# micropilot/myosuite-mjx

Hardware: AMD Instinct MI355X
Metric: env-steps/s (whole node) myoHandPoseRandom-v0 batch 4096 (higher is better)
Workload: dtype f32

## Files before the change

myosuite_mjx_amd/csrc/myo_common.h:

```cpp
#ifndef MYO_COMMON_H
#define MYO_COMMON_H

#include <hip/hip_runtime.h>

#include <algorithm>
#include <utility>
#include <cmath>
#include <cstdint>
#include <cstdio>
#include <cstdlib>
#include <cstring>
#include <mutex>
#include <string>
#include <vector>

#include "../../include/myo_hip.h"

#define MINVALF 1e-15f
#define MAXVALF 1e10f
#define MINIMPF 0.0001f
#define MAXIMPF 0.9999f
#define NCON 32
#define NCAND 128
#ifndef LS_FLOOR
// ... 116 lines not shown

struct TaskDev {
  int task, frame_skip, reset_random, target_generate, ntarget, ntip, obs_dim, nq;
  int tip_site[8];
  float pose_thd, far_th, near_th, w_pose, w_bonus, w_act_reg, w_penalty, w_reach;
  const float *target_lo, *target_hi, *init_qpos, *jnt_lo, *jnt_hi;
  const float* init_qvel;
  const float* rnd;
  float tip_lpos[3];
  int gsize_type;
  float gsize_lo[3], gsize_hi[3];
  const float *init_qpos_alt, *init_qvel_alt;
  float reset_noise_std;
  int fatigue_mode;
  const float* fatigue_vec;
  int terrain, hf_n;
  float terrain_lo, terrain_hi;
  float bd_frame[12];
};

struct DevWalk {
  int obs_dim, hip_period;
  float dt, min_height, max_rot, target_x_vel, target_y_vel;
  float target_rot[4];
  int link_tl, link_tr, link_pel, link_tor;
  float lpos_tl[3], lpos_tr[3], lpos_pel[3], lquat_tor[4];
  int qadr_hfl, qadr_hfr, qadr_ja[4];
  float w_vel, w_done, w_cyc, w_rot, w_ja;
  float mass_total, static_mcom[3];
  float knee_height;
};
enum { KF_AUX = 1, KF_OBS_ONLY = 2, KF_RESET_ONLY = 4 };

__device__ __forceinline__ float dot3(const float* a, const float* b) { return a[0] * b[0] + a[1] * b[1] + a[2] * b[2]; }
__device__ __forceinline__ void cross3(float* r, const float* a, const float* b) {
  float x = a[1] * b[2] - a[2] * b[1], y = a[2] * b[0] - a[0] * b[2], z = a[0] * b[1] - a[1] * b[0];
  r[0] = x; r[1] = y; r[2] = z;
}
__device__ __forceinline__ float norm3(const float* a) { return sqrtf(dot3(a, a)); }
__device__ __forceinline__ float normalize3(float* a) {
  float n = norm3(a);
  if (n < MINVALF) { a[0] = 1; a[1] = 0; a[2] = 0; } else { float i = 1.0f / n; a[0] *= i; a[1] *= i; a[2] *= i; }
  return n;
}
__device__ __forceinline__ float clipf(float x, float lo, float hi) { return fminf(fmaxf(x, lo), hi); }
__device__ __forceinline__ void quat2mat(float* R, const float* q) {
  float w = q[0], x = q[1], y = q[2], z = q[3];
  R[0] = w * w + x * x - y * y - z * z; R[1] = 2 * (x * y - w * z); R[2] = 2 * (x * z + w * y);
  R[3] = 2 * (x * y + w * z); R[4] = w * w - x * x + y * y - z * z; R[5] = 2 * (y * z - w * x);
  R[6] = 2 * (x * z - w * y); R[7] = 2 * (y * z + w * x); R[8] = w * w - x * x - y * y + z * z;
}
__device__ __forceinline__ void euler2quat(float* q, const float* e) {
  float si, ci, sj, cj, sk, ck;
  sincosf(0.5f * e[2], &si, &ci);
  sincosf(-0.5f * e[1], &sj, &cj);
  sincosf(0.5f * e[0], &sk, &ck);
  const float cc = ci * ck, cs = ci * sk, sc = si * ck, ss = si * sk;
  q[0] = cj * cc + sj * ss;
  q[1] = cj * cs - sj * sc;
  q[2] = -(cj * ss + sj * cc);
  q[3] = cj * sc - sj * cs;
}
__device__ __forceinline__ void mulquat(float* r, const float* a, const float* b) {
  float t0 = a[0] * b[0] - a[1] * b[1] - a[2] * b[2] - a[3] * b[3];
  float t1 = a[0] * b[1] + a[1] * b[0] + a[2] * b[3] - a[3] * b[2];
  float t2 = a[0] * b[2] - a[1] * b[3] + a[2] * b[0] + a[3] * b[1];
// ... 83 lines not shown
```

myosuite_mjx_amd/csrc/myo_hip.hip:

```cpp
#include "myo_common.h"
#include "myo_physics.h"
#include "myo_task_track.h"
#include "myo_kernel_lanes.h"
#include "myo_kernel_wave.h"
#include "myo_kernels_aux.h"
#include "myo_host.h"
#include "myo_task_keyturn.h"
#include "myo_task_pen.h"
#include "myo_task_baoding.h"
#include "myo_task_die.h"
#include "myo_task_myodm.h"
#include "myo_host_model.h"

extern "C" {

const char* myo_last_error(void) { return g_err.c_str(); }
int myo_version(void) { return 1; }

int myo_model_load(const void* blobv, size_t nbytes, int device, myo_model** out) {
  if (!blobv || !out || nbytes < 16) return fail(MYO_E_ARG, "myo_model_load: bad arguments");
  const Blob B{(const uint8_t*)blobv};
  uint32_t ver;
  memcpy(&ver, B.p + 4, 4);
  if (memcmp(B.p, "MYOB", 4) || ver != 3) return fail(MYO_E_BLOB, "myo_model_load: not a MYOB v3 blob");
// ... 552 lines not shown
  if (!b) return fail(MYO_E_ARG, "null batch");
  b->env_offset = env_offset;
  b->db.env_offset = env_offset;
  return MYO_OK;
}

int myo_set_state(myo_batch* b, const float* qpos, const float* qvel, const float* act, const float* time, void* stream) {
  if (!b) return fail(MYO_E_ARG, "myo_set_state: null");
  const DevModel& dm = b->model->dm;
  size_t B = b->db.B;
  hipStream_t s = (hipStream_t)stream;
  if (qpos) HIPCHK(hipMemcpyAsync(b->db.qpos, qpos, B * b->model->nq * 4, hipMemcpyDeviceToDevice, s));
  if (qvel) HIPCHK(hipMemcpyAsync(b->db.qvel, qvel, B * dm.nv * 4, hipMemcpyDeviceToDevice, s));
  if (act) HIPCHK(hipMemcpyAsync(b->db.act, act, B * dm.nu * 4, hipMemcpyDeviceToDevice, s));
  if (time) HIPCHK(hipMemcpyAsync(b->db.time, time, B * 4, hipMemcpyDeviceToDevice, s));
  return MYO_OK;
}

#define MYO_WAVE_KERNELS(X)                                                                                             \
  X(WK_HAND, "step_kernel_w<24,8,32,1,3,false,0,false>", 24, 8, 32, 1, 3, false, 0)                                      \
  X(WK_HAND_SPEC, "step_kernel_w<24,8,32,1,4,false,1,false>", 24, 8, 32, 1, 4, false, 1)                                 \
  X(WK_LEG, "step_kernel_w<36,20,32,2,2,false,0,false>", 36, 20, 32, 2, 2, false, 0)                                     \
  X(WK_LEG_SCHED, "step_kernel_w<36,20,32,2,2,true,0,false>", 36, 20, 32, 2, 2, true, 0)                                 \
  X(WK_LEG_SPEC_SCHED, "step_kernel_w<36,20,32,2,2,true,2,false>", 36, 20, 32, 2, 2, true, 2)                            \
  X(WK_LEG_SPEC, "step_kernel_w<36,20,32,2,2,false,2,false>", 36, 20, 32, 2, 2, false, 2)                                \
  X(WK_TERRAIN, "step_kernel_w<36,20,32,2,2,false,0,true>", 36, 20, 32, 2, 2, false, 0, true)                            \
  X(WK_TERRAIN_SPEC_SCHED, "step_kernel_w<36,20,32,2,2,true,3,true>", 36, 20, 32, 2, 2, true, 3, true)                   \
  X(WK_TERRAIN_SPEC, "step_kernel_w<36,20,32,2,2,false,3,true>", 36, 20, 32, 2, 2, false, 3, true)                       \
  X(WK_TRK, "step_kernel_w<36,20,32,2,2,false,0,false,true>", 36, 20, 32, 2, 2, false, 0, false, true)                   \
  X(WK_HAND_RK4, "step_kernel_w<24,8,32,1,3,false,0,false,false,true>", 24, 8, 32, 1, 3, false, 0, false, false, true)   \
  X(WK_LEG_RK4, "step_kernel_w<36,20,32,2,2,false,0,false,false,true>", 36, 20, 32, 2, 2, false, 0, false, false, true)
struct WaveKernel {
  const char* name;
  void (*fn)(const DevModel*, const DevModelW*, DevBatch, const float*, int, int, long long*, const int*, const DevWalk*, int, SchedDev);
};
enum WaveKernelId {
#define X(id, name, ...) id,
  MYO_WAVE_KERNELS(X)
#undef X
};
static const WaveKernel wave_kernels[] = {
#define X(id, name, ...) {name, step_kernel_w<__VA_ARGS__>},
  MYO_WAVE_KERNELS(X)
#undef X
};

static WaveKernelId select_wave_kernel(const myo_model* m, bool bm, bool sched) {
  const bool hand_sizes = m->hand_sizes && !bm, leg_sizes = m->leg_sizes && !bm;
  if (sched) return m->dw.hf.on ? WK_TERRAIN_SPEC_SCHED : (leg_sizes ? WK_LEG_SPEC_SCHED : WK_LEG_SCHED);
  if (m->rk4) return m->wave_cfg == 0 ? WK_HAND_RK4 : WK_LEG_RK4;
  if (m->wave_cfg == 2) return WK_TRK;
  if (m->wave_cfg == 0) return hand_sizes ? WK_HAND_SPEC : WK_HAND;
  if (m->dw.hf.on) return m->terrain_sizes ? WK_TERRAIN_SPEC : WK_TERRAIN;
  return leg_sizes ? WK_LEG_SPEC : WK_LEG;
}

static int launch_step(myo_batch* b, const float* action, int actmap, int nsub, hipStream_t s, int kflags = 0) {
  const myo_model* m = b->model;
  const DevWalk* wk = b->task.task == MYO_TASK_WALK ? b->d_walk : nullptr;
  if (kflags && !(wk && g_lanes == 64)) return fail(MYO_E_ARG, "observation pass: walk task on the wave kernel only");
  const int G = (g_lanes == 64 && !m->wave_ok) ? 16 : ((g_lanes != 64 && !m->generic_ok) ? 64 : g_lanes), EPW = 64 / G;
  int grid = (b->db.B + EPW - 1) / EPW;
  size_t lds = (size_t)EPW * m->env_lds_bytes;
  {
    static std::mutex attr_g_mu;
    static bool attr_g_dev[64] = {};
    std::lock_guard<std::mutex> attr_g_lock(attr_g_mu);
    bool& attr_set = attr_g_dev[m->device & 63];
    if (!attr_set) {
      for (const void* k : {(const void*)step_kernel<16>, (const void*)step_kernel<32>, (const void*)step_kernel<64>, (const void*)reach_obs_kernel<16>})
        HIPCHK(hipFuncSetAttribute(k, hipFuncAttributeMaxDynamicSharedMemorySize, 160 * 1024));
      attr_set = true;
    }
  }
  long long* st = b->d_stamps;
#if MYO_POISON
  {
    static const int pmode = [] { const char* e = getenv("MYO_POISON_MODE"); return e ? atoi(e) : 7; }();
    if (pmode & 1) hipLaunchKernelGGL(scratch_poison_kernel, dim3(16384), dim3(64), 0, s, (float*)b->d_stamps, 0);
    if (pmode & 2) hipLaunchKernelGGL(vgpr_poison_kernel, dim3(8192), dim3(64), 0, s, 0x7fc0dead);
    if (pmode & 4) hipLaunchKernelGGL(sgpr_poison_kernel, dim3(32768), dim3(64), 0, s);
  }
#endif
  if (!(G == 64 && m->wave_ok) && !m->generic_ok)
    return fail(MYO_E_UNSUPPORTED, "this model (tendon limits / free joint / equalities / plane contacts) needs the wave-per-env kernel (lanes = 64)");
  const bool bm = b->bm_on;
  if (bm) {
    int rc = bm_check(b);
    if (rc) return rc;
    const int n = b->db.B * m->dm.nl;
    hipLaunchKernelGGL(link_compose_kernel, dim3((n + 255) / 256), dim3(256), 0, s, b->db, m->dm.nl, m->d_lm_adr, m->d_lm_body, m->d_lm_tab);
// ... 1 lines not shown
  if (G == 64 && m->wave_ok) {
    static std::mutex attr_mu;
    static bool attr_w_dev[64] = {};
    std::lock_guard<std::mutex> attr_lock(attr_mu);
    bool& attr_w = attr_w_dev[m->device & 63];
    if (!attr_w) {
      for (const WaveKernel& k : wave_kernels) HIPCHK(hipFuncSetAttribute((const void*)k.fn, hipFuncAttributeMaxDynamicSharedMemorySize, 64 * 1024));
      attr_w = true;
    }
    const int* order = nullptr;
    int Bn = b->db.B;
    static const int sched_mode = [] { const char* e = getenv("MYO_SCHED"); return e ? atoi(e) : -1; }();
    const int n_cu = m->n_cu > 0 ? m->n_cu : 256;
    const int resident = n_cu * (m->wave_cfg == 0 ? 16 : (m->wave_cfg == 1 ? 8 : std::max(1, (160 * 1024) / std::max(1, m->env_lds_bytes_w))));
    const bool sched_ok = !kflags && Bn >= 64 && Bn <= SCHED_ENV_MASK && nsub + (wk ? 1 : 0) <= 15 && nsub > 0;
    const bool sched = sched_ok && !bm && m->wave_cfg == 1 && !m->rk4 && !(m->dw.hf.on && !m->terrain_sizes) && (sched_mode == 1 || (sched_mode == -1 && m->wave_cfg == 1 && Bn >= 2 * resident));
    if (b->balance && Bn >= 1024 && Bn % 4 == 0 && !kflags && !sched) {
      static const int prio_mode = [] { const char* e = getenv("MYO_PRIO"); return e ? atoi(e) : 2; }();
      hipLaunchKernelGGL(balance_kernel, dim3(1), dim3(1024), 0, s, (const int*)b->db.diag, Bn, b->d_order, Bn / 4, prio_mode);
      order = b->d_order;
    }
    const int nqueue = std::max(1, std::min(8, n_cu / 32));
    SchedDev S{b->d_sched, b->d_sched + 32, nqueue == 8 ? b->sched_stride : (Bn + nqueue - 1) / nqueue + 1, nsub + (wk ? 1 : 0), nqueue};
    const WaveKernel& k = wave_kernels[select_wave_kernel(m, bm, sched)];
    if (!kflags) b->last_kernel = k.name;
    int wgrid = Bn;
    if (sched) {
      hipLaunchKernelGGL(sched_init_kernel, dim3(1), dim3(1024), 0, s, (const int*)b->db.diag, Bn, S);
      wgrid = Bn < resident ? Bn : resident;
      static const int grid_override = [] { const char* e = getenv("MYO_SCHED_GRID"); return e ? atoi(e) : 0; }();
      if (grid_override > 0 && grid_override < wgrid) wgrid = grid_override;
    }
    hipLaunchKernelGGL(k.fn, dim3(wgrid), dim3(64), (size_t)m->env_lds_bytes_w, s, (const DevModel*)m->d_dm, (const DevModelW*)m->d_dw, b->db, action, actmap,
                       nsub, st, order, wk, kflags, S);
    HIPCHK(hipGetLastError());
    return MYO_OK;
  }
  if (G == 16) hipLaunchKernelGGL(step_kernel<16>, dim3(grid), dim3(64), lds, s, m->dm, b->db, action, actmap, nsub, st);
  else if (G == 32) hipLaunchKernelGGL(step_kernel<32>, dim3(grid), dim3(64), lds, s, m->dm, b->db, action, actmap, nsub, st);
  else hipLaunchKernelGGL(step_kernel<64>, dim3(grid), dim3(64), lds, s, m->dm, b->db, action, actmap, nsub, st);
  HIPCHK(hipGetLastError());
  return MYO_OK;
}

int myo_step(myo_batch* b, const float* action_dev, int actmap, int nsubsteps, void* stream) {
  if (!b || nsubsteps < 0) return fail(MYO_E_ARG, "myo_step: bad arguments");
  if (b->task.task == MYO_TASK_TRACK && b->track_flavour == 1 && actmap == MYO_ACTMAP_CTRLRANGE)
    return fail(MYO_E_ARG, "myo_step: MYO_ACTMAP_CTRLRANGE is the MJX TrackEnv's action map; a batch of the classic flavour steps with MYO_ACTMAP_MUSCLE_SIGMOID");
  HIPCHK(hipSetDevice(b->model->device));
  return launch_step(b, action_dev, actmap, nsubsteps, (hipStream_t)stream);
}

static int state_configure(myo_batch* b, const myo_task_config* c) {
  const myo_model* m = b->model;
  const int nv = m->dm.nv, nq = m->nq, na = m->dm.na_obs;
  if (c->task == MYO_TASK_POSE) {
    if (c->ntarget != nv) return fail(MYO_E_ARG, "pose task: ntarget must equal nq");
    b->task.obs_dim = 3 * nv + na;
  } else if (c->task == MYO_TASK_STAND) {
    if (c->ntarget != 3) return fail(MYO_E_ARG, "stand task: ntarget must be 3 (target position)");
    if (!(m->wave_ok && m->dw.has_free && nq == nv + 1)) return fail(MYO_E_UNSUPPORTED, "stand task needs a model with a free root joint");
    b->task.obs_dim = nq + nv + 6 + na;
  } else {
    if (c->ntarget != 3) return fail(MYO_E_ARG, "hold task: ntarget must be 3 (goal position)");
    if (!(m->wave_ok && m->dw.has_free && nq == nv + 1 && nv > 6)) return fail(MYO_E_UNSUPPORTED, "hold task needs a model whose last joint is one free object");
    b->task.obs_dim = (nq - 7) + (nv - 6) + 6 + na;
  }
// ... 94 lines not shown
  HIPCHK(hipGetLastError());
  return MYO_OK;
}

int myo_set_balance(myo_batch* b, int on) {
  if (!b) return fail(MYO_E_ARG, "null batch");
  b->balance = on;
  return MYO_OK;
}

int myo_set_lanes(int lanes) {
  if (lanes != 16 && lanes != 32 && lanes != 64) return fail(MYO_E_ARG, "lanes per env must be 16, 32 or 64");
  g_lanes = lanes;
  return MYO_OK;
}

int myo_read_stamps(myo_batch* b, long long* host, int nwg) {
  if (!b || !host) return fail(MYO_E_ARG, "myo_read_stamps: null");
  HIPCHK(hipDeviceSynchronize());
  HIPCHK(hipMemcpy(host, b->d_stamps, (size_t)nwg * 12 * sizeof(long long), hipMemcpyDeviceToHost));
  return MYO_STAMPS ? MYO_OK : 1;
}

int myo_sync(void* stream) {
  HIPCHK(hipStreamSynchronize((hipStream_t)stream));
  return MYO_OK;
}

int myo_bench_rollout(myo_batch* b, int steps, int nsubsteps, uint64_t seed, int mode, int max_episode_steps, void* stream, float* ms_out) {
  if (!b || steps <= 0) return fail(MYO_E_ARG, "myo_bench_rollout: bad arguments");
  HIPCHK(hipSetDevice(b->model->device));
  hipStream_t s = (hipStream_t)stream;
  int rc;
  if (!(mode & MYO_BENCH_FRESH_ACTIONS)) { rc = myo_random_action(b, b->d_action, seed, b->bench_step, b->env_offset, stream); if (rc) return rc; }
  const int base = ms_out ? 0 : b->kev_pending;
  while ((int)b->kev.size() < 2 * (base + steps)) { hipEvent_t e; HIPCHK(hipEventCreate(&e)); b->kev.push_back(e); }
  if (ms_out) { b->kev_pending = 0; HIPCHK(hipEventRecord(b->ev0, s)); }
  for (int i = 0; i < steps; i++) {
    if (mode & MYO_BENCH_FRESH_ACTIONS) { rc = myo_random_action(b, b->d_action, seed, b->bench_step++, b->env_offset, stream); if (rc) return rc; }
    HIPCHK(hipEventRecord(b->kev[2 * (base + i)], s));
    const bool mjx_track = b->task.task == MYO_TASK_TRACK && b->track_flavour == 0;
    rc = launch_step(b, b->d_action, mjx_track ? MYO_ACTMAP_CTRLRANGE : MYO_ACTMAP_MUSCLE_SIGMOID, nsubsteps, s);
    if (rc) return rc;
    HIPCHK(hipEventRecord(b->kev[2 * (base + i) + 1], s));
    const TaskHooks* hooks = task_hooks(b->task.task);
    if (mjx_track) continue;
    if ((mode & MYO_BENCH_OBS) && (mode & MYO_BENCH_AUTORESET) && max_episode_steps > 0 && hooks && hooks->post) {
      if ((rc = hooks->post(b, s, seed, max_episode_steps))) return rc;
      HIPCHK(hipGetLastError());
      continue;
    }
    if ((mode & MYO_BENCH_OBS) && b->task.task != MYO_TASK_NONE && b->task.task != MYO_TASK_WALK) { rc = launch_obs(b, s); if (rc) return rc; }
    if ((mode & MYO_BENCH_AUTORESET) && max_episode_steps > 0) {
      rc = myo_autoreset(b, max_episode_steps, seed, stream); if (rc) return rc;
      if ((mode & MYO_BENCH_OBS) && b->task.task != MYO_TASK_NONE) { rc = launch_obs(b, s, 1, 1); if (rc) return rc; }
    }
  }
  if (!ms_out) { b->kev_pending = base + steps; return MYO_OK; }
  HIPCHK(hipEventRecord(b->ev1, s));
  HIPCHK(hipEventSynchronize(b->ev1));
  HIPCHK(hipEventElapsedTime(ms_out, b->ev0, b->ev1));
  float tot = 0.f;
  for (int i = 0; i < steps; i++) { float t; HIPCHK(hipEventElapsedTime(&t, b->kev[2 * i], b->kev[2 * i + 1])); tot += t; }
  b->last_kernel_ms = tot;
  return MYO_OK;
}

const char* myo_bench_last_kernel_name(const myo_batch* b) { return b ? b->last_kernel : ""; }

int myo_probe_valu(int device, int waves_per_simd, int iters, double* wave_insts_per_s, int* n_cu_out) {
  if (!wave_insts_per_s || !(waves_per_simd >= 1 && waves_per_simd <= 4 || waves_per_simd == 8) || iters < 1) return fail(MYO_E_ARG, "myo_probe_valu: waves_per_simd must be 1..4 or 8");
  HIPCHK(hipSetDevice(device));
  hipDeviceProp_t prop;
  HIPCHK(hipGetDeviceProperties(&prop, device));
  const int ncu = prop.multiProcessorCount;
  const size_t lds = 60 * 1024;
  HIPCHK(hipFuncSetAttribute((const void*)valu_probe_kernel, hipFuncAttributeMaxDynamicSharedMemorySize, 64 * 1024));
  float* out = nullptr;
  const int wg_per_cu = waves_per_simd == 8 ? 2 : 1;
// ... 92 lines not shown
```

myosuite_mjx_amd/csrc/myo_kernel_wave.h:

```cpp
#ifndef MYO_KERNEL_WAVE_H
#define MYO_KERNEL_WAVE_H

#define NCONW 32
#define MPRW 14
static_assert(4 * MPRW <= 63, "the scheduler carries the table in a 64-word row (word 63 = entry count)");
struct LayW {
  int qpos, qvel, act, ctrl, lpos, lmat, axis, anchor, xv, qfc, sq, mprw, X;
  int tJ, tlen, tforce;
  int cdof, cinert, crb, cvel, cacc, cfrc;
  int gpos, gax, cand, cdist, cpos, cnrm, cpair, cJ, cdofs;
  int Mp;
  int tJp;
  int total;
};
__host__ __device__ constexpr LayW layout_w(int nq, int nv, int nu, int nl, int ngt, int maxnnz, int ncg, bool has_tl, int nvt, int kc, int nc, int nj) {
  LayW Y{};
  int o = 0;
  Y.qpos = o; o += nq; Y.qvel = o; o += nv; Y.act = o; o += nu; Y.ctrl = o; o += nu;
  Y.lpos = o; o += 3 * nl; Y.lmat = o; o += 9 * nl; Y.axis = o; o += 3 * nv; Y.anchor = o; o += 3 * nv;
  Y.xv = o; o += nvt; Y.qfc = o; o += nvt; Y.sq = o; o += nvt * (nvt + 1); Y.mprw = o; o += 4 * MPRW;
  Y.tJp = 0;
  if (has_tl) { Y.tJp = o; o += ngt * maxnnz + 2 * ngt; }
  Y.X = o;
  Y.tJ = o; o += ngt * maxnnz; Y.tlen = o; o += ngt; Y.tforce = o; o += nu;
// ... 313 lines not shown
  __syncthreads();
  if (t == 0) { int acc = 0; for (int k = 0; k < 256; k++) { start[k] = acc; acc += hist[k]; } }
  __syncthreads();
  for (int e = t; e < B; e += 1024) {
    int b = 255 - min(255, (int)(255LL * diag[(size_t)e * 8 + 3] / cmax));
    int r = atomicAdd(&start[b], 1);
    S.ring[(r % nqu) * S.stride + r / nqu] = e;
  }
}

template <int SPEC> struct Sizes { static constexpr int nq = 0, nv = 0, nu = 0, nl = 0, nlevel = 0, maxnnz = 0, nseg = 0, ncg = 0, npair = 0; };
template <> struct Sizes<1> { static constexpr int nq = 23, nv = 23, nu = 39, nl = 17, nlevel = 5, maxnnz = 7, nseg = 116, ncg = 27, npair = 289; };
template <> struct Sizes<2> { static constexpr int nq = 35, nv = 34, nu = 80, nl = 13, nlevel = 6, maxnnz = 11, nseg = 100, ncg = 32, npair = 45; };
template <> struct Sizes<3> { static constexpr int nq = 35, nv = 34, nu = 80, nl = 13, nlevel = 6, maxnnz = 11, nseg = 100, ncg = 33, npair = 76; };
template <int SPEC> static bool sizes_match(int nq, int nv, int nu, int nl, int nlevel, int maxnnz, int ngt, int nseg, int ncg, int npair) {
  typedef Sizes<SPEC> Z;
  return nq == Z::nq && nv == Z::nv && nu == Z::nu && nl == Z::nl && nlevel == Z::nlevel && maxnnz == Z::maxnnz && ngt == Z::nu && nseg == Z::nseg &&
         ncg == Z::ncg && npair == Z::npair;
}

template <int SPEC, int NVT, int KC, int NC, int NJ> struct LayC {
  typedef Sizes<SPEC> Z;
  static constexpr LayW L = layout_w(Z::nq, Z::nv, Z::nu, Z::nl, Z::nu, Z::maxnnz, Z::ncg, false, NVT, KC, NC, NJ);
  static constexpr int qpos = L.qpos, qvel = L.qvel, act = L.act, ctrl = L.ctrl, lpos = L.lpos, lmat = L.lmat, axis = L.axis, anchor = L.anchor, xv = L.xv,
                       qfc = L.qfc, sq = L.sq, mprw = L.mprw, X = L.X, tJ = L.tJ, tlen = L.tlen, tforce = L.tforce, cdof = L.cdof, cinert = L.cinert, crb = L.crb,
                       cvel = L.cvel, cacc = L.cacc, cfrc = L.cfrc, gpos = L.gpos, gax = L.gax, cand = L.cand, cdist = L.cdist, cpos = L.cpos, cnrm = L.cnrm,
                       cpair = L.cpair, cJ = L.cJ, cdofs = L.cdofs, Mp = L.Mp, tJp = L.tJp, total = L.total;
};
template <int SPEC, int NVT, int KC, int NC, int NJ> static bool layout_match(const LayW& a) {
  const LayW b = layout_w(Sizes<SPEC>::nq, Sizes<SPEC>::nv, Sizes<SPEC>::nu, Sizes<SPEC>::nl, Sizes<SPEC>::nu, Sizes<SPEC>::maxnnz, Sizes<SPEC>::ncg, false, NVT, KC, NC, NJ);
  return memcmp(&a, &b, sizeof(LayW)) == 0;
}

template <int NVT, int KC, int NC, int NTR, int WPE, bool SCHED, int SPEC, bool HF = false, bool TRK = false, bool RK4 = false>
__global__ void __launch_bounds__(64, WPE) step_kernel_w(const DevModel* __restrict__ Mp, const DevModelW* __restrict__ Wp, DevBatch Bt,
                                                        const float* __restrict__ action, int actmap, int nsub, long long* stamps,
                                                        const int* __restrict__ order, const DevWalk* __restrict__ wk, int kflags, SchedDev S) {
  extern __shared__ __align__(16) float E[];
  const DevModel& M = *Mp;
  const DevModelW& W = *Wp;
  const LayC<SPEC, NVT, KC, NC, (TRK ? 4 : 3)> Yc{};
  const auto& Y = [&]() -> const auto& { if constexpr (SPEC != 0) return Yc; else return W.lay; }();
#define lane_id wave_lane()
  const int oe = (!SCHED && order) ? order[blockIdx.x] : blockIdx.x;
  int env = oe & 0x0FFFFFFF;
  if (!SCHED) {
    switch (oe >> 28) {
      case 3: __builtin_amdgcn_s_setprio(3); break;
      case 2: __builtin_amdgcn_s_setprio(2); break;
      case 1: __builtin_amdgcn_s_setprio(1); break;
      default: break;
    }
  }
  typedef Sizes<SPEC> Z;
  const int nv = SPEC ? Z::nv : M.nv, nu = SPEC ? Z::nu : M.nu, nq = SPEC ? Z::nq : W.nq;
  const int nl_ = SPEC ? Z::nl : M.nl, nlevel_ = SPEC ? Z::nlevel : M.nlevel, maxnnz_ = SPEC ? Z::maxnnz : M.maxnnz, ngt_ = SPEC ? Z::nu : M.ngt,
            nseg_ = SPEC ? Z::nseg : M.nseg, ncg_ = SPEC ? Z::ncg : M.ncg, npair_ = SPEC ? Z::npair : M.npair;
  constexpr int CDW = (KC + 3) / 4;
  constexpr int NJ = TRK ? 4 : 3;
  constexpr int NR = TRK ? 6 : 4;
  constexpr bool FULL = NVT > 24;
  const bool has_free = FULL && W.has_free;
  const int neq = FULL ? W.neq : 0;
  const bool has_tl = (SPEC != 0 || TRK) ? false : (W.has_tl != 0);
  const bool walk = FULL && wk != nullptr;
  if (!SCHED && FULL && (kflags & KF_RESET_ONLY) && Bt.elapsed[env] != 0) return;
#if MYO_STAMPS
  long long st_acc[12] = {0, 0, 0, 0, 0, 0, 0, 0, 0, 0, 0, 0};
  long long st_t0 = clock64();
  long long st_sub[12] = {0, 0, 0, 0, 0, 0, 0, 0, 0, 0, 0, 0}, st_s0 = 0;
  long long st_x[12] = {0, 0, 0, 0, 0, 0, 0, 0, 0, 0, 0, 0};
#define SUB0() do { st_s0 = clock64(); } while (0)
#define SUB(k) do { long long t1_ = clock64(); st_sub[k] += t1_ - st_s0; st_s0 = t1_; } while (0)
#define SUBX(k) do { long long t1_ = clock64(); st_x[k] += t1_ - st_s0; st_s0 = t1_; } while (0)
#define CNTX(k) do { st_x[k]++; } while (0)
#else
#define SUB0() do { } while (0)
#define SUB(k) do { } while (0)
#define SUBX(k) do { } while (0)
#define CNTX(k) do { } while (0)
#endif
  const int nsubtot = nsub + (walk ? 1 : 0);
  const float h = M.timestep;
  const int sq_q = SCHED ? (int)(__builtin_amdgcn_s_getreg((31 << 11) | 20) & 7) % S.nqueue : 0;
  int* const sq_ctl = SCHED ? S.ctl + 4 * sq_q : nullptr;
  int* const sq_ring = SCHED ? S.ring + (size_t)sq_q * S.stride : nullptr;
  const int sq_n = SCHED ? sq_ctl[2] : 0;
  int last_cost = 0;
  for (;;) {
  int s0 = 0, s1 = nsubtot;
  if (SCHED) {
    int t = 0;
    if (lane_id == 0) t = atomicAdd(&sq_ctl[0], 1);
    t = __builtin_amdgcn_readfirstlane(t);
    if (t >= sq_n * nsubtot) break;
    const int gen = t / sq_n, slot = t - gen * sq_n;
    int v = 0, spins = 0;
    for (;;) {
      v = __hip_atomic_load(&sq_ring[slot], __ATOMIC_RELAXED, __HIP_MEMORY_SCOPE_AGENT);
      if ((v >> 24) == gen || ++spins > (1 << 21)) break;
      __builtin_amdgcn_s_sleep(8);
    }
    v = __builtin_amdgcn_readfirstlane(v);
    if ((v >> 24) != gen) { if (lane_id == 0) { atomicOr(&Bt.flags[0], MYO_FLAG_SCHED_TIMEOUT); sq_ctl[3] = 1; } break; }
    env = v & SCHED_ENV_MASK;
    s0 = (v >> 20) & 15; s1 = s0 + 1;
  }
  float actdot[NTR];
  float* const warm_row = Bt.warm + (size_t)env * nv;
#pragma unroll
  for (int r = 0; r < NTR; r++) actdot[r] = 0.f;
#ifndef MYO_POISON_BITS
#define MYO_POISON_BITS 0x7fc00000
#endif
#if MYO_POISON
  { const int lo_ = MYO_POISON == 1 ? 0 : MYO_POISON == 2 ? 0 : MYO_POISON == 3 ? Y.xv : MYO_POISON == 4 ? Y.sq : MYO_POISON == 5 ? Y.mprw : Y.X;
    const int hi_ = MYO_POISON == 1 ? Y.total : MYO_POISON == 2 ? Y.xv : MYO_POISON == 3 ? Y.sq : MYO_POISON == 4 ? Y.mprw : MYO_POISON == 5 ? Y.X : Y.total;
    for (int i = lo_ + lane_id; i < hi_; i += 64) E[i] = __int_as_float(MYO_POISON_BITS); }
  SYNC();
#endif
  if (lane_id < nq) E[Y.qpos + lane_id] = ldstate<SCHED>(Bt.qpos + (size_t)env * nq + lane_id);
  if (lane_id < nv) {
    E[Y.qvel + lane_id] = ldstate<SCHED>(Bt.qvel + (size_t)env * nv + lane_id);
  }
  for (int i = lane_id; i < nu; i += 64) {
    E[Y.act + i] = ldstate<SCHED>(Bt.act + (size_t)env * nu + i);
    float c;
    if (action && s0 == 0) c = action_map(Bt, M.act, action, env, i, nu, actmap);
    else c = ldstate<SCHED>(Bt.ctrl + (size_t)env * nu + i);
    E[Y.ctrl + i] = c;
  }
  float time = uniformf(ldstate<SCHED>(Bt.time + env));
  const bool track_on = TRK && Bt.track != nullptr && action != nullptr && actmap == MYO_ACTMAP_CTRLRANGE && nsub > 0;
  if constexpr (TRK) { if (track_on) track_lookup(*Bt.track, env, env + Bt.env_offset, time, Bt.elapsed[env], lane_id); }
  int flags = 0, d_nefc = 0, d_ncon = 0, d_iter = 0, d_cost = 0;
  int f_cand = 0, f_mpr = 0, f_ncon = 0, f_iter = 0, f_itcon = 0, f_ls = 0, f_fact = 0;
  if (SCHED && s0 > 0) {
    const int* D = Bt.diag + (size_t)env * 8;
    int a2 = ldstatei<SCHED>(D + 2), a4 = ldstatei<SCHED>(D + 4), a5 = ldstatei<SCHED>(D + 5), a6 = ldstatei<SCHED>(D + 6), a7 = ldstatei<SCHED>(D + 7);
    d_nefc = ldstatei<SCHED>(D); d_ncon = ldstatei<SCHED>(D + 1);
    d_iter = a2; f_cand = a4 & 0xFFFF; f_ncon = a4 >> 16; f_mpr = a5; f_itcon = a6 & 0xFFFF; f_iter = a6 >> 16; f_ls = a7 & 0xFFFF; f_fact = a7 >> 16;
  }
  constexpr bool OVR = FULL && SPEC == 0 && !HF;
  struct PairL { int g1, g2, dl, kc, pt, cd, t1, t2; float margin, gap, rb1, rb2, s1[3], s2[3]; };
  struct PairRaw { float4 q0, q1, q2, q3; };
  auto pair_raw = [&](int p) -> PairRaw { const gpf4 Q = W.pair_rec + 4 * (size_t)p; return PairRaw{Q[0], Q[1], Q[2], Q[3]}; };
  auto pair_decode = [&](const PairRaw& r) -> PairL {
    const float4 q0 = r.q0, q1 = r.q1, q2 = r.q2, q3 = r.q3;
    const int w = __float_as_int(q0.x), tt = __float_as_int(q3.x);
    PairL L;
    L.g1 = w & 255; L.g2 = (w >> 8) & 255; L.pt = (w >> 16) & 15; L.cd = (w >> 20) & 15; L.kc = (w >> 24) & 255; L.dl = __float_as_int(q0.w);
    L.margin = q0.y; L.gap = q0.z; L.t1 = tt & 255; L.t2 = (tt >> 8) & 255;
    L.s1[0] = q1.x; L.s1[1] = q1.y; L.s1[2] = q1.z; L.rb1 = q1.w; L.s2[0] = q2.x; L.s2[1] = q2.y; L.s2[2] = q2.z; L.rb2 = q2.w;
    if (OVR && Bt.gsize) {
      const float* G = Bt.gsize + 4 * (size_t)env;
      if (L.g1 == Bt.gsize_cg) { L.s1[0] = G[0]; L.s1[1] = G[1]; L.s1[2] = G[2]; L.rb1 = G[3]; }
      if (L.g2 == Bt.gsize_cg) { L.s2[0] = G[0]; L.s2[1] = G[1]; L.s2[2] = G[2]; L.rb2 = G[3]; }
    }
    return L;
  };
// ... 1826 lines not shown
      SYNC();
      float* o = Bt.obs + (size_t)env * (nq + nv);
      if (lane_id < nq) o[lane_id] = E[Y.qpos + lane_id];
      if (lane_id < nv) o[nq + lane_id] = E[Y.qvel + lane_id];
    }
  }
  if (lane_id < nq) Bt.qpos[(size_t)env * nq + lane_id] = E[Y.qpos + lane_id];
  if (lane_id < nv) {
    Bt.qvel[(size_t)env * nv + lane_id] = E[Y.qvel + lane_id];
    Bt.qacc[(size_t)env * nv + lane_id] = warm_row[lane_id];
  }
  for (int i = lane_id; i < nu; i += 64) {
    Bt.act[(size_t)env * nu + i] = E[Y.act + i];
    Bt.ctrl[(size_t)env * nu + i] = E[Y.ctrl + i];
  }
  if (SCHED && s1 < nsubtot) {
    int* Wt = Bt.mprw + (size_t)env * 64;
    if (lane_id < 4 * n_mprw) Wt[lane_id] = ((const int*)(E + Y.mprw))[lane_id];
    if (lane_id == 63) Wt[63] = n_mprw;
  }
  if (lane_id == 0) {
    Bt.time[env] = time;
    if (s1 == nsubtot) Bt.elapsed[env] = track_reset ? 0 : Bt.elapsed[env] + 1;
    if (SCHED) { if (flags) atomicOr(&Bt.flags[env], flags); } else Bt.flags[env] |= flags;
    Bt.diag[(size_t)env * 8 + 0] = d_nefc; Bt.diag[(size_t)env * 8 + 1] = d_ncon; Bt.diag[(size_t)env * 8 + 2] = d_iter;
    d_cost = FULL ? 1909 + ((7436 * f_cand - 28892 * f_ncon + 1362 * f_mpr + 25014 * f_iter + 2046 * f_itcon - 1413 * f_ls + 13292 * d_nefc + 343707 * d_ncon) >> 10)
                  : 2236 + ((-141 * f_cand - 3413 * f_ncon + 2188 * f_mpr + 8971 * f_iter - 107 * f_itcon - 122 * f_ls - 518 * d_nefc + 74475 * d_ncon) >> 10);
    d_cost = max(d_cost, 1);
    Bt.diag[(size_t)env * 8 + 3] = d_cost;
    Bt.diag[(size_t)env * 8 + 4] = f_cand | (f_ncon << 16); Bt.diag[(size_t)env * 8 + 5] = f_mpr;
    Bt.diag[(size_t)env * 8 + 6] = f_itcon | (f_iter << 16); Bt.diag[(size_t)env * 8 + 7] = f_ls | (f_fact << 16);
  }
  last_cost = d_cost;
  STAMP(9);
  if (!SCHED) break;
  asm volatile("s_waitcnt vmcnt(0) lgkmcnt(0)" ::: "memory");
  if (s1 < nsubtot && lane_id == 0) {
    const int tt = atomicAdd(&sq_ctl[1], 1);
    const int g2 = tt / sq_n, sl = tt - g2 * sq_n;
    __hip_atomic_store(&sq_ring[sl], (g2 << 24) | (s1 << 20) | env, __ATOMIC_RELAXED, __HIP_MEMORY_SCOPE_AGENT);
  }
  SYNC();
  }
#if MYO_STAMPS
  st_acc[10] = __builtin_amdgcn_s_getreg((31 << 11) | 4);
  st_acc[11] = (__builtin_amdgcn_s_getreg((31 << 11) | 20) & 0xFF) | ((long long)(oe >> 28) << 8) | ((long long)last_cost << 16);
  if (stamps && lane_id == 0) for (int k = 0; k < 12; k++) { stamps[(size_t)blockIdx.x * 12 + k] = st_acc[k]; stamps[((size_t)gridDim.x + blockIdx.x) * 12 + k] = st_sub[k];
                                                stamps[((size_t)2 * gridDim.x + blockIdx.x) * 12 + k] = st_x[k]; }
#endif
}

#undef lane_id
#endif
```

myosuite_mjx_amd/csrc/myo_kernels_aux.h:

```cpp
#ifndef MYO_KERNELS_AUX_H
#define MYO_KERNELS_AUX_H

__global__ void __launch_bounds__(1024) balance_kernel(const int* __restrict__ diag, int B, int* __restrict__ order, int nslot, int prio_mode) {
  __shared__ int hist[256], start[256];
  __shared__ int cmax_s;
  const int t = threadIdx.x;
  if (t < 256) hist[t] = 0;
  if (t == 0) cmax_s = 1;
  __syncthreads();
  int c4[4] = {0, 0, 0, 0};
  int cm = 1;
#pragma unroll
  for (int k = 0; k < 4; k++) { const int e = t + 1024 * k; if (e < B) { c4[k] = diag[(size_t)e * 8 + 3]; cm = max(cm, c4[k]); } }
  for (int e = t + 4096; e < B; e += 1024) cm = max(cm, diag[(size_t)e * 8 + 3]);
  for (int off = 32; off > 0; off >>= 1) cm = max(cm, __shfl_xor(cm, off));
  if ((t & 63) == 0) atomicMax(&cmax_s, cm);
  __syncthreads();
  const float sc = 255.0f / (float)cmax_s;
#define BUCKET(c) (255 - min(255, (int)(sc * (float)(c))))
#pragma unroll
  for (int k = 0; k < 4; k++) if (t + 1024 * k < B) atomicAdd(&hist[BUCKET(c4[k])], 1);
  for (int e = t + 4096; e < B; e += 1024) atomicAdd(&hist[BUCKET(diag[(size_t)e * 8 + 3])], 1);
  __syncthreads();
  if (t < 64) {
// ... 281 lines not shown
    if (obs_only) return;
    float dist = sqrtf(wave_sum(err2));
    float actn = sqrtf(wave_sum(act2)) / (float)(M.na_obs > 0 ? M.na_obs : 1);
    if (lane == 0) {
      float bonus = (dist < 2.f * T.near_th ? 1.f : 0.f) + (dist < T.near_th ? 1.f : 0.f);
      float drop = dist > T.far_th ? 1.f : 0.f;
      Bt.reward[e] = T.w_reach * (-dist) + T.w_bonus * bonus + T.w_act_reg * (-actn) + T.w_penalty * (-drop);
      Bt.solved[e] = dist < T.near_th ? 1.f : 0.f;
      Bt.done[e] = drop;
    }
  }
}
template <void (*Body)(const DevModel&, const DevBatch&, const TaskDev&, int, int, int)>
struct StateObs {
  static __device__ __forceinline__ void obs(const DevModel& M, const DevBatch& Bt, const TaskDev& T, const DevTrack*, uint64_t, int obs_only, int e, int lane) {
    Body(M, Bt, T, obs_only, e, lane);
  }
};
using StateTask = StateObs<obs_body>;
template <void (*Body)(const DevModel&, const DevBatch&, const TaskDev&, const DevTrack&, uint64_t, int, int, int)>
struct TrackObs {
  static __device__ __forceinline__ void obs(const DevModel& M, const DevBatch& Bt, const TaskDev& T, const DevTrack* K, uint64_t seed, int obs_only, int e, int lane) {
    Body(M, Bt, T, *K, seed, obs_only, e, lane);
  }
};
template <class Task>
__global__ void __launch_bounds__(64) task_obs_kernel(DevModel M, DevBatch Bt, TaskDev T, const DevTrack* K, uint64_t seed, int obs_only, int reset_only) {
  const int e = blockIdx.x;
  if (e >= Bt.B) return;
  if (reset_only && Bt.elapsed[e] != 0) return;
  Task::obs(M, Bt, T, K, seed, obs_only, e, threadIdx.x);
}
template <class Task>
__global__ void __launch_bounds__(64) task_post_kernel(DevModel M, DevBatch Bt, TaskDev T, const DevTrack* K, int nq, const float* qpos0, uint64_t seed,
                                                       int env_offset, int auto_max) {
  const int e = blockIdx.x, lane = threadIdx.x;
  if (e >= Bt.B) return;
  Task::obs(M, Bt, T, K, seed, 0, e, lane);
  __syncthreads();
  if (reset_body(Bt, T, nq, M.nv, M.nu, qpos0, nullptr, seed, env_offset, auto_max, e, lane)) {
    __syncthreads();
    Task::obs(M, Bt, T, K, seed, 1, e, lane);
  }
}

template <int G>
__global__ void __launch_bounds__(64) reach_obs_kernel(DevModel M, DevBatch Bt, TaskDev T, int obs_only) {
  extern __shared__ __align__(16) float smem[];
  const Lay& Y = M.lay;
  const int lane = threadIdx.x, grp = lane / G, sub = lane % G;
  int env = blockIdx.x * (64 / G) + grp;
  const bool valid = env < Bt.B;
  if (!valid) env = Bt.B - 1;
  float* E = smem + grp * Y.total;
  const int nv = M.nv, nu = M.nu;
  GFOR(i, nv) E[Y.qpos + i] = Bt.qpos[(size_t)env * nv + i];
  SYNC();
  stage_kinematics<G>(M, E, sub);
  float dt = (float)T.frame_skip * M.timestep;
  float* o = Bt.obs + (size_t)env * T.obs_dim;
  float err2 = 0;
  GFOR(i, T.ntip) {
    float p[3];
    site_world(M, E, T.tip_site[i], p);
    for (int k = 0; k < 3; k++) {
      p[k] += M.origin[k];
      float tg = Bt.target[(size_t)env * T.ntarget + 3 * i + k];
      float re = tg - p[k];
      err2 += re * re;
      if (valid) {
        o[2 * nv + 3 * i + k] = p[k];
        o[2 * nv + 3 * T.ntip + 3 * i + k] = re;
        Bt.sitexpos[(size_t)env * 3 * T.ntip + 3 * i + k] = p[k];
      }
    }
  }
// ... 61 lines not shown
```

myosuite_mjx_amd/csrc/myo_physics.h:

```cpp
#ifndef MYO_PHYSICS_H
#define MYO_PHYSICS_H

__device__ __forceinline__ bool is_intersect(const float* p1, const float* p2, const float* p3, const float* p4) {
  float det = (p4[1] - p3[1]) * (p2[0] - p1[0]) - (p4[0] - p3[0]) * (p2[1] - p1[1]);
  if (fabsf(det) < MINVALF) return false;
  float a = ((p4[0] - p3[0]) * (p1[1] - p3[1]) - (p4[1] - p3[1]) * (p1[0] - p3[0])) / det;
  float b = ((p2[0] - p1[0]) * (p1[1] - p3[1]) - (p2[1] - p1[1]) * (p1[0] - p3[0])) / det;
  return a >= 0 && a <= 1 && b >= 0 && b <= 1;
}

__device__ float wrap_circle(float* pnt, const float* d, const float* sd, bool has_side, float rad) {
  float sq0 = d[0] * d[0] + d[1] * d[1], sq1 = d[2] * d[2] + d[3] * d[3], sqr = rad * rad;
  if (sq0 < sqr || sq1 < sqr || rad < MINVALF) return -1;
  float dif[2] = {d[2] - d[0], d[3] - d[1]};
  float dd = dif[0] * dif[0] + dif[1] * dif[1];
  if (dd < MINVALF) return -1;
  float a = clipf(-(dif[0] * d[0] + dif[1] * d[1]) / dd, 0.f, 1.f);
  float tmp[2] = {a * dif[0] + d[0], a * dif[1] + d[1]};
  if (tmp[0] * tmp[0] + tmp[1] * tmp[1] > sqr && (!has_side || sd[0] * tmp[0] + sd[1] * tmp[1] >= 0)) return -1;
  float s0 = sqrtf(sq0 - sqr), s1 = sqrtf(sq1 - sqr);
  float sol[2][4], good[2];
  bool crossing[2];
#pragma unroll
  for (int i = 0; i < 2; i++) {
// ... 188 lines not shown

__device__ __forceinline__ float muscle_fl(float L, float lmin, float lmax) {
  if (lmin <= L && L <= lmax) {
    float a = 0.5f * (lmin + 1), b = 0.5f * (1 + lmax), x;
    if (L <= a) { x = (L - lmin) / fmaxf(MINVALF, a - lmin); return 0.5f * x * x; }
    else if (L <= 1) { x = (1 - L) / fmaxf(MINVALF, 1 - a); return 1 - 0.5f * x * x; }
    else if (L <= b) { x = (L - 1) / fmaxf(MINVALF, b - 1); return 1 - 0.5f * x * x; }
    else { x = (lmax - L) / fmaxf(MINVALF, lmax - b); return 0.5f * x * x; }
  }
  return 0;
}
__device__ __forceinline__ void muscle(const float* A, float len, float vel, float act, float ctrl, float* force, float* actdot) {
  float r0 = A[0], r1 = A[1], F0 = A[2], lmin = A[3], lmax = A[4], vmax = A[5], fpmax = A[6], fvmax = A[7], lr0 = A[8], lr1 = A[9];
  float L0 = (lr1 - lr0) / fmaxf(MINVALF, r1 - r0);
  float L = r0 + (len - lr0) / fmaxf(MINVALF, L0);
  float V = vel / fmaxf(MINVALF, L0 * vmax);
  float FL = muscle_fl(L, lmin, lmax), FV, y = fvmax - 1;
  if (V <= -1) FV = 0;
  else if (V <= 0) FV = (V + 1) * (V + 1);
  else if (V <= y) FV = fvmax - (y - V) * (y - V) / fmaxf(MINVALF, y);
  else FV = fvmax;
  float gain = -F0 * FL * FV;
  float b = 0.5f * (1 + lmax), bias, x;
  if (L <= 1) bias = 0;
  else if (L <= b) { x = (L - 1) / fmaxf(MINVALF, b - 1); bias = -A[15] * fpmax * 0.5f * x * x; }
  else { x = (L - b) / fmaxf(MINVALF, b - 1); bias = -A[15] * fpmax * (0.5f + x); }
  *force = gain * act + bias;
  float cc = clipf(clipf(ctrl, A[12], A[13]), 0.f, 1.f), ac = clipf(act, 0.f, 1.f);
  float tau_act = A[10] * (0.5f + 1.5f * ac), tau_deact = A[11] / (0.5f + 1.5f * ac);
  float dctrl = cc - act;
  *actdot = dctrl / fmaxf(MINVALF, dctrl > 0 ? tau_act : tau_deact);
}

__device__ __forceinline__ float action_map(const DevBatch& Bt, const float* __restrict__ actprm, const float* __restrict__ action, int env,
                                            int i, int nu, int actmap) {
  int src = i;
  if (actmap == MYO_ACTMAP_SIGMOID_REAFFERENTATION) { if (i == Bt.reaf_epl) src = Bt.reaf_eip; else if (i == Bt.reaf_eip) return 0.f; }
  float c = action[(size_t)env * nu + src];
  if (actmap == MYO_ACTMAP_NONE) return c;
  if (actmap == MYO_ACTMAP_CTRLRANGE) {
    const DevTrack* K = Bt.track;
    const float t = (c + 1.0f) * (K->hi[i] - K->lo[i]) * 0.5f;
    return t + K->lo[i];
  }
  if (actprm[16 * i + 10] < 0.f) return actprm[16 * i + 6] + c * actprm[16 * i + 5];
  c = 1.0f / (1.0f + expf(-5.0f * (c - 0.5f)));
  if (actmap == MYO_ACTMAP_SIGMOID_FATIGUE) {
    float* S = Bt.fatigue + (size_t)env * 3 * nu;
    float MA = S[i], MR = S[nu + i], MF = S[2 * nu + i];
    const float F = 0.00912f, R = 0.1f * 0.00094f, rr = 10.f * 15.f, dt = Bt.fat_dt, TL = c;
    float LD = (0.5f + 1.5f * MA) / actprm[16 * i + 10], LR = (0.5f + 1.5f * MA) / actprm[16 * i + 11];
    float C, rR;
    if (MA < TL) { C = (MR > TL - MA) ? LD * (TL - MA) : LD * MR; rR = R; }
    else { C = LR * (TL - MA); rR = rr * R; }
    float lo = fmaxf(-MA / dt + F * MA, (MR - 1) / dt + rR * MF), hi = fminf((1 - MA) / dt + F * MA, MR / dt + rR * MF);
    C = fminf(fmaxf(C, lo), hi);
    S[i] = MA + (C - F * MA) * dt;
    S[nu + i] = MR + (-C + rR * MF) * dt;
    S[2 * nu + i] = MF + (F * MA - rR * MF) * dt;
    c = S[i];
  }
  return c;
}

__device__ __forceinline__ float impedance(const float* solimp, float pos, float margin) {
  float dmin = clipf(solimp[0], MINIMPF, MAXIMPF), dmax = clipf(solimp[1], MINIMPF, MAXIMPF);
  float width = fmaxf(MINVALF, solimp[2]), mid = clipf(solimp[3], MINIMPF, MAXIMPF), power = fmaxf(1.f, solimp[4]);
  if (dmin == dmax || width <= MINVALF) return 0.5f * (dmin + dmax);
  float x = fabsf((pos - margin) / width);
  if (x >= 1) return dmax;
  if (x == 0) return dmin;
  float y;
  if (power == 1) y = x;
  else if (power == 2) y = x <= mid ? x * x / mid : 1 - (1 - x) * (1 - x) / (1 - mid);
  else if (x <= mid) y = powf(x, power) / powf(mid, power - 1);
  else y = 1 - powf(1 - x, power) / powf(1 - mid, power - 1);
  return dmin + y * (dmax - dmin);
}
__device__ __forceinline__ void kbi(float solref0, float solref1, float dmax_in, float timestep, float* K, float* B) {
  float dmax = clipf(dmax_in, MINIMPF, MAXIMPF);
  if (solref0 > 0) {
    float tc = fmaxf(solref0, 2 * timestep);
    *K = 1.0f / fmaxf(MINVALF, dmax * dmax * tc * tc * solref1 * solref1);
    *B = 2.0f / fmaxf(MINVALF, dmax * tc);
  } else {
    *K = -solref0 / fmaxf(MINVALF, dmax * dmax);
    *B = -solref1 / fmaxf(MINVALF, dmax);
  }
}

__device__ __forceinline__ void make_frame(const float* n, float* t1, float* t2) {
  t1[0] = 0; t1[1] = 0; t1[2] = 0;
  if (n[1] < 0.5f && n[1] > -0.5f) t1[1] = 1; else t1[2] = 1;
  float t = dot3(n, t1);
  t1[0] -= t * n[0]; t1[1] -= t * n[1]; t1[2] -= t * n[2];
// ... 391 lines not shown
```

Baseline: 4.461 million.

## Fuse random action draw and state-task post/reset into hand wave step kernel

For the 24-dof hand wave kernel, random actions are now drawn inside the step kernel instead of by a separate random-action launch. The per-step observation and autoreset post kernel for state tasks also runs at the end of the step kernel. This removes two kernel launches per env step and the global-memory round trip of the action buffer. In exchange the step kernel carries more code and register pressure, and it adds a wait plus a workgroup barrier before the post stage.

Measured after the change: 4.428 million. About the same (-0.7%).

```diff
diff --git a/myosuite_mjx_amd/csrc/myo_common.h b/myosuite_mjx_amd/csrc/myo_common.h
--- a/myosuite_mjx_amd/csrc/myo_common.h
+++ b/myosuite_mjx_amd/csrc/myo_common.h
@@ -172,6 +172,15 @@
 };
 enum { KF_AUX = 1, KF_OBS_ONLY = 2, KF_RESET_ONLY = 4 };
 
+enum { SF_DRAW = 1, SF_POST = 2 };
+struct StepFuse {
+  int mode;
+  int auto_max;
+  uint64_t seed, step;
+  float* action_out;
+  TaskDev T;
+};
+
 __device__ __forceinline__ float dot3(const float* a, const float* b) { return a[0] * b[0] + a[1] * b[1] + a[2] * b[2]; }
 __device__ __forceinline__ void cross3(float* r, const float* a, const float* b) {
   float x = a[1] * b[2] - a[2] * b[1], y = a[2] * b[0] - a[0] * b[2], z = a[0] * b[1] - a[1] * b[0];
diff --git a/myosuite_mjx_amd/csrc/myo_hip.hip b/myosuite_mjx_amd/csrc/myo_hip.hip
--- a/myosuite_mjx_amd/csrc/myo_hip.hip
+++ b/myosuite_mjx_amd/csrc/myo_hip.hip
@@ -608,7 +608,7 @@
   X(WK_LEG_RK4, "step_kernel_w<36,20,32,2,2,false,0,false,false,true>", 36, 20, 32, 2, 2, false, 0, false, false, true)
 struct WaveKernel {
   const char* name;
-  void (*fn)(const DevModel*, const DevModelW*, DevBatch, const float*, int, int, long long*, const int*, const DevWalk*, int, SchedDev);
+  void (*fn)(const DevModel*, const DevModelW*, DevBatch, const float*, int, int, long long*, const int*, const DevWalk*, int, SchedDev, StepFuse);
 };
 enum WaveKernelId {
 #define X(id, name, ...) id,
@@ -631,8 +631,11 @@
   return leg_sizes ? WK_LEG_SPEC : WK_LEG;
 }
 
-static int launch_step(myo_batch* b, const float* action, int actmap, int nsub, hipStream_t s, int kflags = 0) {
+static bool step_fusable(const myo_batch* b) { return g_lanes == 64 && b->model->wave_ok && b->model->wave_cfg == 0; }
+
+static int launch_step(myo_batch* b, const float* action, int actmap, int nsub, hipStream_t s, int kflags = 0, const StepFuse* fuse = nullptr) {
   const myo_model* m = b->model;
+  if (fuse && (kflags || !step_fusable(b))) return fail(MYO_E_ARG, "fused env step: plain step launches of the 24-dof wave kernels only");
   const DevWalk* wk = b->task.task == MYO_TASK_WALK ? b->d_walk : nullptr;
   if (kflags && !(wk && g_lanes == 64)) return fail(MYO_E_ARG, "observation pass: walk task on the wave kernel only");
   const int G = (g_lanes == 64 && !m->wave_ok) ? 16 : ((g_lanes != 64 && !m->generic_ok) ? 64 : g_lanes), EPW = 64 / G;
@@ -700,7 +703,7 @@
       if (grid_override > 0 && grid_override < wgrid) wgrid = grid_override;
     }
     hipLaunchKernelGGL(k.fn, dim3(wgrid), dim3(64), (size_t)m->env_lds_bytes_w, s, (const DevModel*)m->d_dm, (const DevModelW*)m->d_dw, b->db, action, actmap,
-                       nsub, st, order, wk, kflags, S);
+                       nsub, st, order, wk, kflags, S, fuse ? *fuse : StepFuse{});
     HIPCHK(hipGetLastError());
     return MYO_OK;
   }
@@ -861,19 +864,28 @@
   HIPCHK(hipSetDevice(b->model->device));
   hipStream_t s = (hipStream_t)stream;
   int rc;
+  const char* fe = getenv("MYO_FUSED_STEP");
+  const bool fusable = !(fe && atoi(fe) == 0) && step_fusable(b);
+  const TaskHooks* const hooks = task_hooks(b->task.task);
+  StepFuse fuse{};
+  if (fusable && (mode & MYO_BENCH_FRESH_ACTIONS)) { fuse.mode |= SF_DRAW; fuse.seed = seed; fuse.action_out = b->d_action; }
+  if (fusable && hooks == &state_hooks && (mode & MYO_BENCH_OBS) && (mode & MYO_BENCH_AUTORESET) && max_episode_steps > 0) {
+    fuse.mode |= SF_POST; fuse.seed = seed; fuse.auto_max = max_episode_steps; fuse.T = b->task;
+  }
   if (!(mode & MYO_BENCH_FRESH_ACTIONS)) { rc = myo_random_action(b, b->d_action, seed, b->bench_step, b->env_offset, stream); if (rc) return rc; }
   const int base = ms_out ? 0 : b->kev_pending;
   while ((int)b->kev.size() < 2 * (base + steps)) { hipEvent_t e; HIPCHK(hipEventCreate(&e)); b->kev.push_back(e); }
   if (ms_out) { b->kev_pending = 0; HIPCHK(hipEventRecord(b->ev0, s)); }
   for (int i = 0; i < steps; i++) {
-    if (mode & MYO_BENCH_FRESH_ACTIONS) { rc = myo_random_action(b, b->d_action, seed, b->bench_step++, b->env_offset, stream); if (rc) return rc; }
+    if (fuse.mode & SF_DRAW) fuse.step = b->bench_step++;
+    else if (mode & MYO_BENCH_FRESH_ACTIONS) { rc = myo_random_action(b, b->d_action, seed, b->bench_step++, b->env_offset, stream); if (rc) return rc; }
     HIPCHK(hipEventRecord(b->kev[2 * (base + i)], s));
     const bool mjx_track = b->task.task == MYO_TASK_TRACK && b->track_flavour == 0;
-    rc = launch_step(b, b->d_action, mjx_track ? MYO_ACTMAP_CTRLRANGE : MYO_ACTMAP_MUSCLE_SIGMOID, nsubsteps, s);
+    rc = launch_step(b, (fuse.mode & SF_DRAW) ? nullptr : b->d_action, mjx_track ? MYO_ACTMAP_CTRLRANGE : MYO_ACTMAP_MUSCLE_SIGMOID, nsubsteps, s, 0,
+                     fuse.mode ? &fuse : nullptr);
     if (rc) return rc;
     HIPCHK(hipEventRecord(b->kev[2 * (base + i) + 1], s));
-    const TaskHooks* hooks = task_hooks(b->task.task);
-    if (mjx_track) continue;
+    if (mjx_track || (fuse.mode & SF_POST)) continue;
     if ((mode & MYO_BENCH_OBS) && (mode & MYO_BENCH_AUTORESET) && max_episode_steps > 0 && hooks && hooks->post) {
       if ((rc = hooks->post(b, s, seed, max_episode_steps))) return rc;
       HIPCHK(hipGetLastError());
diff --git a/myosuite_mjx_amd/csrc/myo_kernel_wave.h b/myosuite_mjx_amd/csrc/myo_kernel_wave.h
--- a/myosuite_mjx_amd/csrc/myo_kernel_wave.h
+++ b/myosuite_mjx_amd/csrc/myo_kernel_wave.h
@@ -369,10 +369,14 @@
   return memcmp(&a, &b, sizeof(LayW)) == 0;
 }
 
+__device__ __forceinline__ void fused_state_post(const DevModel& M, const DevBatch& Bt, const TaskDev& T, int nq, const float* qpos0, uint64_t seed,
+                                                 int auto_max, int e, int lane);
+
 template <int NVT, int KC, int NC, int NTR, int WPE, bool SCHED, int SPEC, bool HF = false, bool TRK = false, bool RK4 = false>
 __global__ void __launch_bounds__(64, WPE) step_kernel_w(const DevModel* __restrict__ Mp, const DevModelW* __restrict__ Wp, DevBatch Bt,
                                                         const float* __restrict__ action, int actmap, int nsub, long long* stamps,
-                                                        const int* __restrict__ order, const DevWalk* __restrict__ wk, int kflags, SchedDev S) {
+                                                        const int* __restrict__ order, const DevWalk* __restrict__ wk, int kflags, SchedDev S,
+                                                        StepFuse F) {
   extern __shared__ __align__(16) float E[];
   const DevModel& M = *Mp;
   const DevModelW& W = *Wp;
@@ -397,6 +401,8 @@
   constexpr int NJ = TRK ? 4 : 3;
   constexpr int NR = TRK ? 6 : 4;
   constexpr bool FULL = NVT > 24;
+  constexpr bool FUSE = !FULL && !SCHED && !TRK;
+  const bool draw = FUSE && (F.mode & SF_DRAW);
   const bool has_free = FULL && W.has_free;
   const int neq = FULL ? W.neq : 0;
   const bool has_tl = (SPEC != 0 || TRK) ? false : (W.has_tl != 0);
@@ -463,6 +469,12 @@
   for (int i = lane_id; i < nu; i += 64) {
     E[Y.act + i] = ldstate<SCHED>(Bt.act + (size_t)env * nu + i);
     float c;
+    if (FUSE && draw) {
+      const uint64_t key = (uint64_t)(env + Bt.env_offset) * 1024;
+      auto drawn = [&](int k) { return 2.0f * u01(F.seed, key + k, F.step) - 1.0f; };
+      if (F.action_out) F.action_out[(size_t)env * nu + i] = drawn(i);
+      c = action_map(Bt, M.act, nullptr, env, i, nu, actmap, drawn);
+    } else
     if (action && s0 == 0) c = action_map(Bt, M.act, action, env, i, nu, actmap);
     else c = ldstate<SCHED>(Bt.ctrl + (size_t)env * nu + i);
     E[Y.ctrl + i] = c;
@@ -2355,6 +2367,13 @@
     Bt.diag[(size_t)env * 8 + 6] = f_itcon | (f_iter << 16); Bt.diag[(size_t)env * 8 + 7] = f_ls | (f_fact << 16);
   }
   last_cost = d_cost;
+  if constexpr (FUSE) {
+    if (F.mode & SF_POST) {
+      asm volatile("s_waitcnt vmcnt(0) lgkmcnt(0)" ::: "memory");
+      SYNC();
+      fused_state_post(M, Bt, F.T, nq, (const float*)M.qpos0, F.seed, F.auto_max, env, lane_id);
+    }
+  }
   STAMP(9);
   if (!SCHED) break;
   asm volatile("s_waitcnt vmcnt(0) lgkmcnt(0)" ::: "memory");
diff --git a/myosuite_mjx_amd/csrc/myo_kernels_aux.h b/myosuite_mjx_amd/csrc/myo_kernels_aux.h
--- a/myosuite_mjx_amd/csrc/myo_kernels_aux.h
+++ b/myosuite_mjx_amd/csrc/myo_kernels_aux.h
@@ -337,16 +337,25 @@
   Task::obs(M, Bt, T, K, seed, obs_only, e, threadIdx.x);
 }
 template <class Task>
+__device__ __forceinline__ void task_post_body(const DevModel& M, const DevBatch& Bt, const TaskDev& T, const DevTrack* K, int nq, const float* qpos0,
+                                               uint64_t seed, int env_offset, int auto_max, const int e, const int lane) {
+  Task::obs(M, Bt, T, K, seed, 0, e, lane);
+  __syncthreads();
+  if (reset_body(Bt, T, nq, M.nv, M.nu, qpos0, nullptr, seed, env_offset, auto_max, e, lane)) {
+    __syncthreads();
+    Task::obs(M, Bt, T, K, seed, 1, e, lane);
+  }
+}
+template <class Task>
 __global__ void __launch_bounds__(64) task_post_kernel(DevModel M, DevBatch Bt, TaskDev T, const DevTrack* K, int nq, const float* qpos0, uint64_t seed,
                                                        int env_offset, int auto_max) {
   const int e = blockIdx.x, lane = threadIdx.x;
   if (e >= Bt.B) return;
-  Task::obs(M, Bt, T, K, seed, 0, e, lane);
-  __syncthreads();
-  if (reset_body(Bt, T, nq, M.nv, M.nu, qpos0, nullptr, seed, env_offset, auto_max, e, lane)) {
-    __syncthreads();
-    Task::obs(M, Bt, T, K, seed, 1, e, lane);
-  }
+  task_post_body<Task>(M, Bt, T, K, nq, qpos0, seed, env_offset, auto_max, e, lane);
+}
+__device__ __forceinline__ void fused_state_post(const DevModel& M, const DevBatch& Bt, const TaskDev& T, int nq, const float* qpos0, uint64_t seed,
+                                                 int auto_max, int e, int lane) {
+  task_post_body<StateTask>(M, Bt, T, nullptr, nq, qpos0, seed, Bt.env_offset, auto_max, e, lane);
 }
 
 template <int G>
diff --git a/myosuite_mjx_amd/csrc/myo_physics.h b/myosuite_mjx_amd/csrc/myo_physics.h
--- a/myosuite_mjx_amd/csrc/myo_physics.h
+++ b/myosuite_mjx_amd/csrc/myo_physics.h
@@ -244,11 +244,12 @@
   *actdot = dctrl / fmaxf(MINVALF, dctrl > 0 ? tau_act : tau_deact);
 }
 
+template <class Draw>
 __device__ __forceinline__ float action_map(const DevBatch& Bt, const float* __restrict__ actprm, const float* __restrict__ action, int env,
-                                            int i, int nu, int actmap) {
+                                            int i, int nu, int actmap, Draw draw) {
   int src = i;
   if (actmap == MYO_ACTMAP_SIGMOID_REAFFERENTATION) { if (i == Bt.reaf_epl) src = Bt.reaf_eip; else if (i == Bt.reaf_eip) return 0.f; }
-  float c = action[(size_t)env * nu + src];
+  float c = action ? action[(size_t)env * nu + src] : draw(src);
   if (actmap == MYO_ACTMAP_NONE) return c;
   if (actmap == MYO_ACTMAP_CTRLRANGE) {
     const DevTrack* K = Bt.track;
@@ -273,6 +274,10 @@
     c = S[i];
   }
   return c;
+}
+__device__ __forceinline__ float action_map(const DevBatch& Bt, const float* __restrict__ actprm, const float* __restrict__ action, int env,
+                                            int i, int nu, int actmap) {
+  return action_map(Bt, actprm, action, env, i, nu, actmap, [](int) { return 0.f; });
 }
 
 __device__ __forceinline__ float impedance(const float* solimp, float pos, float margin) {
```
